# dfm/george

Hardware: NVIDIA H100
Metric: gp.compute+log_likelihood N-points/sec (higher is better)
Workload: dtype f64

## Files before the change

### george_b200/csrc/hodlr_leaf.cuh

```cuda
#pragma once

#include "gemm_dmma.cuh"
#include "hodlr_kernels.cuh"

namespace bgp {

constexpr int LF_THREADS = 256;
constexpr int LF_NB = 32;
constexpr int LF_MAX_LEAF = 768;

__host__ __device__ inline int lf_panel_ld(int max_m) { return ((max_m + 15) / 16) * 16 + 4; }

template <int SHAPE>
__global__ void __launch_bounds__(LF_THREADS, 2) leaf_factor_kernel(const DevProgram* __restrict__ gprog,
                                                                    const double* __restrict__ x,
                                                                    const double* __restrict__ diag,
                                                                    const LeafDesc* __restrict__ leaves,
                                                                    double* __restrict__ Lbuf,
                                                                    double* __restrict__ leaf_logdet, int ldp) {
  extern __shared__ __align__(16) double lf_smem[];
  double* pn = lf_smem;
  double* dall = lf_smem + LF_NB * ldp;
  DevProgram* P = reinterpret_cast<DevProgram*>(lf_smem + (LF_NB + 1) * ldp);
  __shared__ double red[32];
  __shared__ double dinv[LF_NB];
  if constexpr (SHAPE == BGP_SHAPE_GENERIC) stage_program(P, gprog);
  __syncthreads();
  const auto fn = ShapeEval<SHAPE>::make(P, gprog);
  const LeafDesc lf = leaves[blockIdx.x];
  const int m = lf.size, nd = gprog->ndim;
  double* A = Lbuf + lf.off;
  const double* xs = x + (int64_t)lf.start * nd;
  const int lane = threadIdx.x & 31, warp = threadIdx.x >> 5;

  double logdet = 0.0;
  for (int k0 = 0; k0 < m; k0 += LF_NB) {
    const int nb = min(LF_NB, m - k0), rem = m - k0;
    for (int t = threadIdx.x; t < nb * rem; t += LF_THREADS) {
      const int c = t / rem, i = t - c * rem;
      if (i >= c) {
        double v = fn(xs + (int64_t)(k0 + i) * nd, xs + (int64_t)(k0 + c) * nd);
        if (i == c) v += diag[lf.start + k0 + i];
        pn[c * ldp + i] = v;
      }
    }
    __syncthreads();
    if (k0 > 0) {
      const int lr = lane >> 2, lc = lane & 3;
      const int n_tiles = (rem + 15) / 16;
      bool bok[4];
#pragma unroll
      for (int b = 0; b < 4; ++b) bok[b] = b * 8 + lr < nb;
      for (int t = warp; t < n_tiles; t += LF_THREADS / 32) {
        const int r0 = t * 16;
        bool aok[2];
#pragma unroll
        for (int a = 0; a < 2; ++a) aok[a] = r0 + a * 8 + lr < rem;
        double acc[2][4][2];
#pragma unroll
        for (int a = 0; a < 2; ++a)
#pragma unroll
          for (int b = 0; b < 4; ++b) { acc[a][b][0] = 0.0; acc[a][b][1] = 0.0; }
#pragma unroll 4
        for (int q0 = 0; q0 < k0; q0 += 4) {
          const int q = q0 + lc;
          const double* Lq = A + (int64_t)q * m + k0;
          const double dq = dall[q];
          double af[2], bf[4];
#pragma unroll
          for (int a = 0; a < 2; ++a) af[a] = aok[a] ? Lq[r0 + a * 8 + lr] : 0.0;
#pragma unroll
          for (int b = 0; b < 4; ++b) bf[b] = bok[b] ? Lq[b * 8 + lr] * dq : 0.0;
#pragma unroll
          for (int a = 0; a < 2; ++a)
#pragma unroll
            for (int b = 0; b < 4; ++b) dmma884(acc[a][b][0], acc[a][b][1], af[a], bf[b]);
        }
#pragma unroll
        for (int a = 0; a < 2; ++a) {
          const int i = r0 + a * 8 + lr;
#pragma unroll
          for (int b = 0; b < 4; ++b)
#pragma unroll
            for (int e = 0; e < 2; ++e) {
              const int c = b * 8 + 2 * lc + e;
              if (i < rem && c < nb && i >= c) pn[c * ldp + i] -= acc[a][b][e];
            }
        }
      }
      __syncthreads();
    }
    if (warp == 0) {
      double w[LF_NB];
#pragma unroll
      for (int j = 0; j < LF_NB; ++j) w[j] = (j <= lane && lane < nb) ? pn[j * ldp + lane] : 0.0;
#pragma unroll
      for (int k = 0; k < LF_NB; ++k) {
        if (k < nb) {
          const double d = __shfl_sync(0xffffffffu, w[k], k);
          const double l = (lane > k && lane < nb) ? w[k] / d : 0.0;
          if (lane > k) w[k] = l;
          const double ld = l * d;
#pragma unroll
          for (int j = k + 1; j < LF_NB; ++j) {
            const double lj = __shfl_sync(0xffffffffu, l, j);
            if (j <= lane) w[j] -= ld * lj;
          }
        }
      }
      if (lane < nb) {
        double* col = A + (int64_t)k0 * m + k0 + lane;
        double d = 0.0;
#pragma unroll
        for (int j = 0; j < LF_NB; ++j) {
          if (j < lane) { pn[j * ldp + lane] = w[j]; col[(int64_t)j * m] = w[j]; }
          if (j == lane) d = w[j];
        }
        col[(int64_t)lane * m] = d;
        dall[k0 + lane] = d;
        dinv[lane] = 1.0 / d;
        logdet += log(fabs(d));
      }
    }
    __syncthreads();
    const volatile double* l11 = pn;
    for (int i = LF_NB + threadIdx.x; i < rem; i += LF_THREADS) {
      double w[LF_NB];
#pragma unroll
      for (int j = 0; j < LF_NB; ++j) w[j] = pn[j * ldp + i];
#pragma unroll
      for (int j = 0; j < LF_NB; ++j) {
        double s = w[j];
#pragma unroll
        for (int q = 0; q < j; ++q) s -= w[q] * l11[q * ldp + j];
        w[j] = s;
      }
      double* row = A + (int64_t)k0 * m + k0 + i;
#pragma unroll
      for (int j = 0; j < LF_NB; ++j) row[(int64_t)j * m] = w[j] * dinv[j];
    }
    __syncthreads();
  }
  logdet = block_sum(logdet, red);
  if (threadIdx.x == 0) leaf_logdet[blockIdx.x] = logdet;
}

__host__ inline size_t lf_smem_bytes(int shape, int max_m) {
  return sizeof(double) * (size_t)(LF_NB + 1) * lf_panel_ld(max_m) + (shape == BGP_SHAPE_GENERIC ? sizeof(DevProgram) : 0);
}

template <int SHAPE>
inline void leaf_factor_launch_shape(int n_leaves, int max_m, cudaStream_t s, const DevProgram* prog, const double* x,
                                     const double* diag, const LeafDesc* leaves, double* L, double* leaf_logdet) {
  const size_t smem = lf_smem_bytes(SHAPE, max_m);
  cudaFuncSetAttribute(leaf_factor_kernel<SHAPE>, cudaFuncAttributeMaxDynamicSharedMemorySize, (int)smem);
  leaf_factor_kernel<SHAPE><<<n_leaves, LF_THREADS, smem, s>>>(prog, x, diag, leaves, L, leaf_logdet, lf_panel_ld(max_m));
}

inline void leaf_factor_launch(int shape, int n_leaves, int max_m, cudaStream_t s, const DevProgram* prog,
                               const double* x, const double* diag, const LeafDesc* leaves, double* L,
                               double* leaf_logdet) {
  BGP_SHAPE_SWITCH(shape, (leaf_factor_launch_shape<SHAPE>(n_leaves, max_m, s, prog, x, diag, leaves, L, leaf_logdet)));
}

}
```

Measured before the change: 22.34 million.

## Replace per-row panel triangular solve with inverse-L11 DMMA multiply in leaf factor

The diagonal 32x32 block factorization now runs in shared memory and also builds an explicit inverse of the unit-lower factor scaled by 1/D. The off-diagonal panel solve then becomes a tensor-core DMMA product against that inverse, replacing the per-thread serial forward substitution over 32 columns. Kernel-matrix panel construction is additionally unrolled by 4 for non-generic shapes to expose ILP. The panel padding grows and shared memory use increases, and explicit inversion may slightly change numerics.

```diff
diff --git a/george_b200/csrc/hodlr_leaf.cuh b/george_b200/csrc/hodlr_leaf.cuh
--- a/george_b200/csrc/hodlr_leaf.cuh
+++ b/george_b200/csrc/hodlr_leaf.cuh
@@ -8,8 +8,21 @@
 constexpr int LF_THREADS = 256;
 constexpr int LF_NB = 32;
 constexpr int LF_MAX_LEAF = 768;
-
-__host__ __device__ inline int lf_panel_ld(int max_m) { return ((max_m + 15) / 16) * 16 + 4; }
+constexpr int LF_LDW = 40;
+
+__host__ __device__ inline int lf_panel_ld(int max_m) { return ((max_m + 15) / 16) * 16 + 8; }
+
+__device__ __forceinline__ void lf_axpy(double* dst, int ds, const double* src, int ss, int lo, int hi, double f) {
+  for (int j0 = lo; j0 <= hi; j0 += 8) {
+    double a[8], b[8];
+#pragma unroll
+    for (int u = 0; u < 8; ++u)
+      if (j0 + u <= hi) { a[u] = dst[(j0 + u) * ds]; b[u] = src[(j0 + u) * ss]; }
+#pragma unroll
+    for (int u = 0; u < 8; ++u)
+      if (j0 + u <= hi) dst[(j0 + u) * ds] = a[u] - f * b[u];
+  }
+}
 
 template <int SHAPE>
 __global__ void __launch_bounds__(LF_THREADS, 2) leaf_factor_kernel(const DevProgram* __restrict__ gprog,
@@ -21,9 +34,9 @@
   extern __shared__ __align__(16) double lf_smem[];
   double* pn = lf_smem;
   double* dall = lf_smem + LF_NB * ldp;
-  DevProgram* P = reinterpret_cast<DevProgram*>(lf_smem + (LF_NB + 1) * ldp);
+  double* w11 = dall + ldp;
+  DevProgram* P = reinterpret_cast<DevProgram*>(w11 + LF_NB * LF_LDW);
   __shared__ double red[32];
-  __shared__ double dinv[LF_NB];
   if constexpr (SHAPE == BGP_SHAPE_GENERIC) stage_program(P, gprog);
   __syncthreads();
   const auto fn = ShapeEval<SHAPE>::make(P, gprog);
@@ -32,21 +45,27 @@
   double* A = Lbuf + lf.off;
   const double* xs = x + (int64_t)lf.start * nd;
   const int lane = threadIdx.x & 31, warp = threadIdx.x >> 5;
-
+  const int lr = lane >> 2, lc = lane & 3;
+
+  constexpr int LF_BUILD_ILP = SHAPE == BGP_SHAPE_GENERIC ? 1 : 4;
   double logdet = 0.0;
   for (int k0 = 0; k0 < m; k0 += LF_NB) {
     const int nb = min(LF_NB, m - k0), rem = m - k0;
-    for (int t = threadIdx.x; t < nb * rem; t += LF_THREADS) {
-      const int c = t / rem, i = t - c * rem;
-      if (i >= c) {
-        double v = fn(xs + (int64_t)(k0 + i) * nd, xs + (int64_t)(k0 + c) * nd);
-        if (i == c) v += diag[lf.start + k0 + i];
-        pn[c * ldp + i] = v;
+    for (int t0 = threadIdx.x; t0 < nb * rem; t0 += LF_BUILD_ILP * LF_THREADS) {
+      double v[LF_BUILD_ILP];
+#pragma unroll
+      for (int u = 0; u < LF_BUILD_ILP; ++u) {
+        const int t = t0 + u * LF_THREADS, c = t / rem, i = t - c * rem;
+        v[u] = (t < nb * rem && i >= c) ? fn(xs + (int64_t)(k0 + i) * nd, xs + (int64_t)(k0 + c) * nd) : 0.0;
+      }
+#pragma unroll
+      for (int u = 0; u < LF_BUILD_ILP; ++u) {
+        const int t = t0 + u * LF_THREADS, c = t / rem, i = t - c * rem;
+        if (t < nb * rem && i >= c) pn[c * ldp + i] = (i == c) ? v[u] + diag[lf.start + k0 + i] : v[u];
       }
     }
     __syncthreads();
     if (k0 > 0) {
-      const int lr = lane >> 2, lc = lane & 3;
       const int n_tiles = (rem + 15) / 16;
       bool bok[4];
 #pragma unroll
@@ -91,53 +110,70 @@
       __syncthreads();
     }
     if (warp == 0) {
-      double w[LF_NB];
-#pragma unroll
-      for (int j = 0; j < LF_NB; ++j) w[j] = (j <= lane && lane < nb) ? pn[j * ldp + lane] : 0.0;
-#pragma unroll
-      for (int k = 0; k < LF_NB; ++k) {
-        if (k < nb) {
-          const double d = __shfl_sync(0xffffffffu, w[k], k);
-          const double l = (lane > k && lane < nb) ? w[k] / d : 0.0;
-          if (lane > k) w[k] = l;
+      double* t11 = w11;
+      for (int j = 0; j < LF_NB; ++j) t11[j * LF_LDW + lane] = (j == lane) ? 1.0 : 0.0;
+      __syncwarp();
+      for (int k = 0; k < nb; ++k) {
+        const double d = pn[k * ldp + k];
+        const bool below = lane > k && lane < nb;
+        const double l = below ? pn[k * ldp + lane] / d : 0.0;
+        if (below) pn[k * ldp + lane] = l;
+        __syncwarp();
+        if (below) {
           const double ld = l * d;
-#pragma unroll
-          for (int j = k + 1; j < LF_NB; ++j) {
-            const double lj = __shfl_sync(0xffffffffu, l, j);
-            if (j <= lane) w[j] -= ld * lj;
-          }
-        }
+          lf_axpy(pn + lane, ldp, pn + k * ldp, 1, k + 1, lane, ld);
+          lf_axpy(t11 + lane, LF_LDW, t11 + k, LF_LDW, 0, k, l);
+        }
+        __syncwarp();
       }
       if (lane < nb) {
+        const double d = pn[lane * ldp + lane];
+        const double dinv = 1.0 / d;
         double* col = A + (int64_t)k0 * m + k0 + lane;
-        double d = 0.0;
-#pragma unroll
-        for (int j = 0; j < LF_NB; ++j) {
-          if (j < lane) { pn[j * ldp + lane] = w[j]; col[(int64_t)j * m] = w[j]; }
-          if (j == lane) d = w[j];
-        }
+        for (int j = 0; j < lane; ++j) col[(int64_t)j * m] = pn[j * ldp + lane];
         col[(int64_t)lane * m] = d;
         dall[k0 + lane] = d;
-        dinv[lane] = 1.0 / d;
         logdet += log(fabs(d));
+        for (int j = 0; j <= lane; ++j) t11[j * LF_LDW + lane] *= dinv;
       }
     }
     __syncthreads();
-    const volatile double* l11 = pn;
-    for (int i = LF_NB + threadIdx.x; i < rem; i += LF_THREADS) {
-      double w[LF_NB];
-#pragma unroll
-      for (int j = 0; j < LF_NB; ++j) w[j] = pn[j * ldp + i];
-#pragma unroll
-      for (int j = 0; j < LF_NB; ++j) {
-        double s = w[j];
-#pragma unroll
-        for (int q = 0; q < j; ++q) s -= w[q] * l11[q * ldp + j];
-        w[j] = s;
-      }
-      double* row = A + (int64_t)k0 * m + k0 + i;
-#pragma unroll
-      for (int j = 0; j < LF_NB; ++j) row[(int64_t)j * m] = w[j] * dinv[j];
+    if (rem > LF_NB) {
+      const int n_tiles = (rem - LF_NB + 15) / 16;
+      for (int t = warp; t < n_tiles; t += LF_THREADS / 32) {
+        const int r0 = LF_NB + t * 16;
+        bool aok[2];
+#pragma unroll
+        for (int a = 0; a < 2; ++a) aok[a] = r0 + a * 8 + lr < rem;
+        double acc[2][4][2];
+#pragma unroll
+        for (int a = 0; a < 2; ++a)
+#pragma unroll
+          for (int b = 0; b < 4; ++b) { acc[a][b][0] = 0.0; acc[a][b][1] = 0.0; }
+#pragma unroll
+        for (int q0 = 0; q0 < LF_NB; q0 += 4) {
+          const int q = q0 + lc;
+          double af[2], bf[4];
+#pragma unroll
+          for (int a = 0; a < 2; ++a) af[a] = aok[a] ? pn[q * ldp + r0 + a * 8 + lr] : 0.0;
+#pragma unroll
+          for (int b = 0; b < 4; ++b) bf[b] = w11[q * LF_LDW + b * 8 + lr];
+#pragma unroll
+          for (int a = 0; a < 2; ++a)
+#pragma unroll
+            for (int b = 0; b < 4; ++b) dmma884(acc[a][b][0], acc[a][b][1], af[a], bf[b]);
+        }
+#pragma unroll
+        for (int a = 0; a < 2; ++a) {
+          const int i = r0 + a * 8 + lr;
+          if (i < rem) {
+#pragma unroll
+            for (int b = 0; b < 4; ++b)
+#pragma unroll
+              for (int e = 0; e < 2; ++e) A[(int64_t)(k0 + b * 8 + 2 * lc + e) * m + k0 + i] = acc[a][b][e];
+          }
+        }
+      }
     }
     __syncthreads();
   }
@@ -146,7 +182,8 @@
 }
 
 __host__ inline size_t lf_smem_bytes(int shape, int max_m) {
-  return sizeof(double) * (size_t)(LF_NB + 1) * lf_panel_ld(max_m) + (shape == BGP_SHAPE_GENERIC ? sizeof(DevProgram) : 0);
+  return sizeof(double) * ((size_t)(LF_NB + 1) * lf_panel_ld(max_m) + LF_NB * LF_LDW) +
+         (shape == BGP_SHAPE_GENERIC ? sizeof(DevProgram) : 0);
 }
 
 template <int SHAPE>
```

Result: faster. 23.29 million, median of 6 (+4.3%).
